# lars-frogner/Impact

Measured on AMD Instinct MI355X. Metric: voxels stepped/sec + remesh tris/sec, 512^3 grid, 1/2/4/8 MI355X, higher is better.
Workload: dtype i8 voxels, f32 SDF/mesh arithmetic, f64 moments; 1 GPU; config-2 SDF asteroid x2.05 -> 502^3 grid = 512^3 stored voxels (32768 chunks); parallelism=single GPU, voxels_per_gpu=134217728, regions=1, triangles=1813104

## Files before the change

impact_amd/csrc/sn_roles.hpp:

```cpp
#pragma once
#include "ivx_internal.hpp"

namespace ivx_roles {
namespace sn {


constexpr int G = 18, NROWS = 324, NCROWS = 289, NCUBES = 4913;
constexpr int RS = 24, TILE_BYTES = NROWS * RS;
constexpr uint32_t VPC = 864;
__device__ __forceinline__ int tix(int a, int b, int c) { return (a * G + b) * RS + 3 + c; }

__device__ __forceinline__ uint32_t opaque(uint32_t x) {
    asm volatile("" : "+v"(x));
    return x;
}
struct V3 {
    float x, y, z;
};
__device__ __forceinline__ V3 mk(float x, float y, float z) { return V3{x, y, z}; }
__device__ __forceinline__ V3 add(V3 a, V3 b) { return {a.x + b.x, a.y + b.y, a.z + b.z}; }
__device__ __forceinline__ V3 sub(V3 a, V3 b) { return {a.x - b.x, a.y - b.y, a.z - b.z}; }
__device__ __forceinline__ V3 mul(V3 a, V3 b) { return {a.x * b.x, a.y * b.y, a.z * b.z}; }
__device__ __forceinline__ V3 scale(V3 a, float s) { return {a.x * s, a.y * s, a.z * s}; }
__device__ __forceinline__ float len3(V3 a) { return sqrtf((a.x * a.x + a.y * a.y) + a.z * a.z); }
__device__ __forceinline__ bool sneg(float f) { return (__float_as_uint(f) >> 31) != 0; }
__device__ __forceinline__ float decode(int8_t e) { return (float)e * 0.02f; }

struct SnParams {
    GridView g;
    float extent;
    uint32_t x_off;
};

struct RowLoads {
    uint32_t c0, c1, c2;
    uint4 s4, t4;
    uint32_t b0s, b0t, b2s, b2t;
};
__device__ __forceinline__ uint32_t row_mode(const GridView& g, int gi, int gj) {
    if (gj < 0 || gj >= (int)g.cy * 16) return 0u;
    if (gi < 0 || gi >= (int)g.cx * 16) return 2u;
    return 1u;
}
__device__ __forceinline__ void row_issue(const GridView& g, int gi, int gj, int ck, RowLoads& L) {
    if (row_mode(g, gi, gj) != 1u) return;
    const size_t cidx = (size_t)(((gi >> 4) * g.cy + (gj >> 4)) * g.cz) + (size_t)ck;
    const uint32_t rix = (uint32_t)(((gi & 15) << 4) | (gj & 15));
    const size_t o = (cidx << 12) + ((size_t)rix << 4);
    const bool has_lo = ck > 0, has_hi = ck + 1 < (int)g.cz;
    const uint32_t* ip = reinterpret_cast<const uint32_t*>(g.info + cidx);
    const uint8_t* kf = g.kface + cidx * 1024 + rix;
    const uint32_t* ip0 = has_lo ? ip - 2 : ip;
    const uint32_t* ip2 = has_hi ? ip + 2 : ip;
    const uint8_t* kf0 = has_lo ? kf - 1024 : kf;
// ... 837 lines not shown
        if ((any & bit) == 0u) continue;
        const bool crossed = (cm & bit) != 0u;
        const float q = div_ranged(d[c1], d[c1] - d[c2]);
        const float t = crossed ? q : 0.0f;
        const float s = crossed ? ((1.0f - q) + q) : 0.0f;
        sum.x += axis == 4 ? t : ((c1 & 4) ? s : 0.0f);
        sum.y += axis == 2 ? t : ((c1 & 2) ? s : 0.0f);
        sum.z += axis == 1 ? t : ((c1 & 1) ? s : 0.0f);
    }
}

struct RowData {
    uint4 s4, t4;
    uint32_t b0s, b0t, b2s, b2t;
};
struct TileLoads {
    RowData L[2];
    uint32_t rec;
};
__device__ __forceinline__ void rim_row(int h, int& a, int& b) {
    a = h < 18 ? 0 : (h < 36 ? G - 1 : 1 + ((h - 36) >> 1));
    b = h < 18 ? h : (h < 36 ? h - 18 : ((h & 1) ? G - 1 : 0));
}
__device__ __forceinline__ void tile_issue(const GridView& g, uint32_t chunk, TileLoads& T, uint32_t tid) {
    tid = opaque(tid);
    const int ck = chunk % g.cz, cj = (chunk / g.cz) % g.cy, ci = chunk / (g.cz * g.cy);
    T.rec = 0u;
    if (tid < 27u) {
        const int di = (int)(tid / 9u) - 1, dj = (int)((tid / 3u) % 3u) - 1, dk = (int)(tid % 3u) - 1;
        const int ni = ci + di, nj = cj + dj, nk = ck + dk;
        if (nj >= 0 && nj < (int)g.cy && nk >= 0 && nk < (int)g.cz) {
            const ivx_chunk_info* rp = nullptr;
            if (ni >= 0 && ni < (int)g.cx) rp = g.info + (size_t)((ni * (int)g.cy + nj) * (int)g.cz + nk);
            else if (g.ghost_info[ni < 0 ? 0 : 1]) rp = g.ghost_info[ni < 0 ? 0 : 1] + (nj * (int)g.cz + nk);
            if (rp) T.rec = *reinterpret_cast<const uint32_t*>(rp);
        }
    }
    {
        RowData& L = T.L[0];
        const size_t o = ((size_t)chunk << 12) + ((size_t)tid << 4);
        const uint32_t* kf = reinterpret_cast<const uint32_t*>(g.kface + (size_t)chunk * 1024) + (tid >> 2);
        const uint32_t* kf0 = ck > 0 ? kf - 256 : kf;
        const uint32_t* kf2 = ck + 1 < (int)g.cz ? kf + 256 : kf;
        L.s4 = *reinterpret_cast<const uint4*>(g.sdf + o);
        L.t4 = *reinterpret_cast<const uint4*>(g.type + o);
        L.b0s = kf0[64];
        L.b0t = kf0[192];
        L.b2s = kf2[0];
        L.b2t = kf2[128];
    }
    {
        RowData& L = T.L[1];
        int a, b;
        rim_row((int)tid, a, b);
        int gi = ci * 16 + a - 1, gj = cj * 16 + b - 1;
        const bool real = tid < 68u && row_mode(g, gi, gj) == 1u;
        gi = real ? gi : ci * 16;
        gj = real ? gj : cj * 16;
        const size_t cidx = (size_t)(((gi >> 4) * g.cy + (gj >> 4)) * g.cz) + (size_t)ck;
        const uint32_t rix = (uint32_t)(((gi & 15) << 4) | (gj & 15));
        const size_t o = (cidx << 12) + ((size_t)rix << 4);
        const uint32_t* kf = reinterpret_cast<const uint32_t*>(g.kface + cidx * 1024) + (rix >> 2);
        const uint32_t* kf0 = ck > 0 ? kf - 256 : kf;
        const uint32_t* kf2 = ck + 1 < (int)g.cz ? kf + 256 : kf;
        L.s4 = *reinterpret_cast<const uint4*>(g.sdf + o);
        L.t4 = *reinterpret_cast<const uint4*>(g.type + o);
        L.b0s = kf0[64];
        L.b0t = kf0[192];
        L.b2s = kf2[0];
        L.b2t = kf2[128];
    }
}
__device__ __forceinline__ void tile_pin(TileLoads& T) {
#pragma unroll
    for (int r = 0; r < 2; ++r) {
        RowData& L = T.L[r];
        asm volatile("" : "+v"(L.s4.x), "+v"(L.s4.y), "+v"(L.s4.z), "+v"(L.s4.w), "+v"(L.t4.x), "+v"(L.t4.y), "+v"(L.t4.z), "+v"(L.t4.w));
        asm volatile("" : "+v"(L.b0s), "+v"(L.b0t), "+v"(L.b2s), "+v"(L.b2t));
    }
    asm volatile("" : "+v"(T.rec));
}
__device__ __forceinline__ void tile_records(TileLoads& T, uint32_t* s_rec, uint32_t tid) {
    if (tid < 27u) s_rec[tid] = T.rec;
}
__device__ __forceinline__ void tile_row_store(RowData& L, uint32_t rix, uint32_t w0, uint32_t w1, uint32_t w2, bool has_lo, bool has_hi, uint32_t sd[6],
                                               uint32_t ty[6]) {
    asm volatile("" : "+v"(L.s4.x), "+v"(L.s4.y), "+v"(L.s4.z), "+v"(L.s4.w), "+v"(L.t4.x), "+v"(L.t4.y), "+v"(L.t4.z), "+v"(L.t4.w));
    asm volatile("" : "+v"(L.b0s), "+v"(L.b0t), "+v"(L.b2s), "+v"(L.b2t));
    const ivx_chunk_info c0 = record_of(w0), c1 = record_of(w1), c2 = record_of(w2);
    const bool d1 = c1.kind == KIND_NONUNIFORM;
    const uint32_t us = ivx_uniform_sdf(c1.kind) * 0x01010101u, ut = ivx_uniform_type(c1) * 0x01010101u;
    sd[1] = d1 ? L.s4.x : us, sd[2] = d1 ? L.s4.y : us, sd[3] = d1 ? L.s4.z : us, sd[4] = d1 ? L.s4.w : us;
    ty[1] = d1 ? L.t4.x : ut, ty[2] = d1 ? L.t4.y : ut, ty[3] = d1 ? L.t4.z : ut, ty[4] = d1 ? L.t4.w : ut;
    const uint32_t sh = 8u * (rix & 3u);
    if (has_lo) {
        const bool dense = c0.kind == KIND_NONUNIFORM;
        sd[0] = dense ? ((L.b0s >> sh) & 0xFFu) : ivx_uniform_sdf(c0.kind);
        ty[0] = dense ? ((L.b0t >> sh) & 0xFFu) : ivx_uniform_type(c0);
    }
    if (has_hi) {
        const bool dense = c2.kind == KIND_NONUNIFORM;
        sd[5] = dense ? ((L.b2s >> sh) & 0xFFu) : ivx_uniform_sdf(c2.kind);
        ty[5] = dense ? ((L.b2t >> sh) & 0xFFu) : ivx_uniform_type(c2);
    }
}
__device__ __forceinline__ void tile_row_write(int r, const uint32_t sd[6], const uint32_t ty[6], uint8_t* s_sd, uint8_t* s_ty, uint32_t* s_neg) {
    s_neg[r] = ((sd[0] >> 7) & 1u) | (neg16(sd + 1) << 1) | (((sd[5] >> 7) & 1u) << 17);
    uint8_t* ds = s_sd + r * RS;
    uint8_t* dt = s_ty + r * RS;
    ds[3] = (uint8_t)sd[0];
    dt[3] = (uint8_t)ty[0];
#pragma unroll
    for (int q = 0; q < 4; ++q) {
        reinterpret_cast<uint32_t*>(ds + 4)[q] = sd[1 + q];
        reinterpret_cast<uint32_t*>(dt + 4)[q] = ty[1 + q];
    }
    ds[20] = (uint8_t)sd[5];
    dt[20] = (uint8_t)ty[5];
}
__device__ __forceinline__ void tile_finish(const GridView& g, uint32_t chunk, TileLoads& T, const uint32_t* s_rec, uint8_t* s_sd, uint8_t* s_ty, uint32_t* s_neg,
                                            uint32_t tid, int* upper) {
    tid = opaque(tid);
    const int ck = chunk % g.cz, cj = (chunk / g.cz) % g.cy, ci = chunk / (g.cz * g.cy);
    const bool has_lo = ck > 0, has_hi = ck + 1 < (int)g.cz;
    {
        uint32_t sd[6], ty[6];
        sd[0] = sd[5] = 0x7Fu;
        ty[0] = ty[5] = 0xFFu;
        tile_row_store(T.L[0], tid, s_rec[12], s_rec[13], s_rec[14], has_lo, has_hi, sd, ty);
        tile_row_write((int)(((tid >> 4) + 1u) * G + (tid & 15u) + 1u), sd, ty, s_sd, s_ty, s_neg);
    }
    if (tid < 68u) {
        int a, b;
        rim_row((int)tid, a, b);
        const int gi = ci * 16 + a - 1, gj = cj * 16 + b - 1;
        uint32_t sd[6], ty[6];
        sd[0] = sd[5] = 0x7Fu;
        ty[0] = ty[5] = 0xFFu;
        sd[1] = sd[2] = sd[3] = sd[4] = 0x7F7F7F7Fu;
        ty[1] = ty[2] = ty[3] = ty[4] = 0xFFFFFFFFu;
        const uint32_t mode = row_mode(g, gi, gj);
        if (mode == 2u) {
            fetch_row_serial(g, gi, gj, ck, sd, ty);
        } else if (mode == 1u) {
            const int col = (((gi >> 4) - ci + 1) * 3 + ((gj >> 4) - cj + 1)) * 3;
            tile_row_store(T.L[1], (uint32_t)(((gi & 15) << 4) | (gj & 15)), s_rec[col], s_rec[col + 1], s_rec[col + 2], has_lo, has_hi, sd, ty);
        }
        tile_row_write(a * G + b, sd, ty, s_sd, s_ty, s_neg);
    }
    upper[0] = upper[1] = upper[2] = G - 1;
    if ((s_rec[22] & 0xFFu) == KIND_NONUNIFORM) upper[0] -= 1;
    if ((s_rec[16] & 0xFFu) == KIND_NONUNIFORM) upper[1] -= 1;
    if ((s_rec[14] & 0xFFu) == KIND_NONUNIFORM) upper[2] -= 1;
}

static inline uint32_t ivx_emit_grid(const ivx_grid* g, uint32_t n_entries) {
    const uint32_t resident = (uint32_t)g->ctx->n_cu * 4u;
    return n_entries < resident ? (n_entries ? n_entries : 1u) : resident;
}
static inline uint32_t ivx_emit_general_grid(const ivx_grid* g, uint32_t n_entries) {
    const uint32_t cap = (uint32_t)g->ctx->n_cu * 2u;
    return n_entries < cap ? (n_entries ? n_entries : 1u) : cap;
}

#define IVX_MESH_ST(p, v) __builtin_nontemporal_store((v), (p))
template <bool SLOTS>
__device__ __forceinline__ void role_sn_emit(uint32_t bid, uint32_t nb, SnParams p, float* __restrict__ positions, float* __restrict__ normals,
                                                 uint32_t* __restrict__ indices, unsigned long long* __restrict__ imats, ivx_submesh* __restrict__ submeshes,
                                                 const uint32_t* __restrict__ emit_count, const uint4* __restrict__ emit_items, uint32_t vcap, uint32_t icap,
                                                 uint32_t scap, const uint32_t* __restrict__ slots, uint32_t* __restrict__ hard_count,
                                                 uint32_t* __restrict__ hard_list, uint32_t* __restrict__ cursor, SnWalk walk = SnWalk{nullptr, nullptr, nullptr, 0u},
                                                 uint32_t walk_len = 0u) {
    __shared__ uint16_t s_quad[3 * VPC];
    __shared__ __attribute__((aligned(16))) uint8_t s_sd[TILE_BYTES];
    __shared__ __attribute__((aligned(16))) uint8_t s_ty[TILE_BYTES];
    __shared__ uint32_t s_neg2[2][NROWS];
    __shared__ uint32_t s_vrow[NCROWS];
    __shared__ uint16_t s_qrow[NCROWS];
    __shared__ uint2 s_qbits[NCROWS];
    __shared__ uint32_t s_nq;
    __shared__ uint16_t s_surf[VPC];
    __shared__ float s_vpos[3][VPC];
    __shared__ uint8_t s_vsm[VPC];
    __shared__ uint32_t s_wsum[4];
    __shared__ uint32_t s_hard;
    __shared__ uint32_t s_rec[27];
    __shared__ uint32_t s_ticket[5];
    __shared__ float s_rcount[13];
    const GridView& g = p.g;
    const uint32_t tid = threadIdx.x;
    if (tid >= 1u && tid < 13u) s_rcount[tid] = 1.0f / (float)tid;
    const uint32_t n_emit = emit_count[0];
    constexpr uint32_t NONE = 0xFFFFFFFFu;
    const uint32_t walk_front = walk.items ? walk.count[0] : 0u;
    uint32_t li = NONE, li_next = bid, li_prev = NONE;
    if (li_next >= n_emit) return;
    uint4 item = make_uint4(0u, 0u, 0u, 0u), item_next;
    if (walk.items) {
        const uint32_t w = bid < walk_front ? bid : walk_len - 1u - (bid - walk_front);
        item_next = walk.items[w];
        li_next = walk.li[w];
    } else {
        item_next = emit_items[li_next];
    }
    int upper[3] = {G - 1, G - 1, G - 1};
    uint32_t info_w = 0u;
// ... 17 lines not shown
        sm.chunk_indices[0] = (uint32_t)ci + p.x_off;
        sm.chunk_indices[1] = (uint32_t)cj;
        sm.chunk_indices[2] = (uint32_t)ck;
        sm.index_offset = ioff;
        sm.index_count = icount;
        for (int a = 0; a < 2; ++a)
            for (int b = 0; b < 2; ++b)
                for (int c = 0; c < 2; ++c)
                    sm.is_obscured_from_direction[a][b][c] =
                        (((cflags >> (3 * a)) & 1u) && ((cflags >> (3 * b + 1)) & 1u) && ((cflags >> (3 * c + 2)) & 1u)) ? 1u : 0u;
        sm.vertex_offset = voff;
        sm.vertex_count = item.w & 0xFFFFu;
        sm.reserved = 0;
        submeshes[slot] = sm;
    }
    __syncthreads();
    if (have) IVX_T(g, li, 1);
    if (from_ticket) {
        li_next = (uint32_t)__builtin_amdgcn_readfirstlane((int)s_ticket[0]);
        item_next = make_uint4((uint32_t)__builtin_amdgcn_readfirstlane((int)s_ticket[1]), (uint32_t)__builtin_amdgcn_readfirstlane((int)s_ticket[2]),
                               (uint32_t)__builtin_amdgcn_readfirstlane((int)s_ticket[3]), (uint32_t)__builtin_amdgcn_readfirstlane((int)s_ticket[4]));
    }
    const bool have_next = li_next < n_emit;
    if (tid == 0) {
        if (li_prev != NONE && s_hard) hard_list[atomicAdd(hard_count, 1u)] = li_prev;
        s_hard = large ? 1u : 0u;
    }

    uint32_t ticket = 0u;
    if (tid == TK && have_next) ticket = nb + 8u * atomicAdd(cursor + 32u * (bid & 7u), 1u) + (bid & 7u);
    TileLoads T;
    if (have_next) tile_issue(g, item_next.x, T, tid);
    uint4 drawn = make_uint4(0u, 0u, 0u, 0u);
    uint32_t drawn_li = 0u;
    {
        uint32_t vb[2] = {0, 0}, nq[2] = {0, 0};
        const int r0 = 2 * (int)opaque(tid);
        for (int q = 0; q < 2; ++q) {
            const int cr = r0 + q;
            if (cr < NCROWS) {
                uint32_t qx, qy, qz;
                cube_row_bits(s_neg, cr / 17, cr % 17, upper, vb[q], qx, qy, qz);
                nq[q] = __popc(qx) + __popc(qy) + __popc(qz);
                s_qbits[cr] = make_uint2(qx | (qy << 17), (qy >> 15) | (qz << 2));
            }
        }
        uint32_t total;
        const uint32_t pre = block_prefix<false>((__popc(vb[0]) + __popc(vb[1])) | ((nq[0] + nq[1]) << 16), s_wsum, tid, total);
        uint32_t base = pre & 0xFFFFu, qb = pre >> 16;
        if (tid == 0) s_nq = total >> 16;
        for (int q = 0; q < 2; ++q) {
            const int cr = r0 + q;
            if (cr < NCROWS) {
                s_vrow[cr] = (base << 17) | vb[q];
                s_qrow[cr] = (uint16_t)qb;
                qb += nq[q];
                uint32_t m = vb[q];
                while (m) {
                    const int k = __ffs(m) - 1;
                    m &= m - 1;
                    if (base < VPC) s_surf[base] = (uint16_t)(cr * 17 + k);
                    base += 1;
                }
            }
        }
    }
    if (have_next) tile_pin(T);
    if (have) IVX_T(g, li, 6);
    __syncthreads();
    if (have) IVX_T(g, li, 2);
    if ((tid >> 6) == (TK >> 6)) {
        const uint32_t tk = (uint32_t)__builtin_amdgcn_readfirstlane((int)ticket);
        if (have_next && tk < n_emit) {
            if (walk.items) {
                const uint32_t w = tk < walk_front ? tk : walk_len - 1u - (tk - walk_front);
                drawn = walk.items[w];
                drawn_li = walk.li[w];
            } else {
                drawn = emit_items[tk];
                drawn_li = tk;
            }
            asm volatile("" : "+v"(drawn.x), "+v"(drawn.y), "+v"(drawn.z), "+v"(drawn.w), "+v"(drawn_li));
        } else {
            drawn_li = tk;
        }
    }

    const float chunk_extent = p.extent * 16.0f;
    const V3 pos_offset = mk((float)(ci + (int)p.x_off) * chunk_extent - 0.5f * p.extent, (float)cj * chunk_extent - 0.5f * p.extent,
                             (float)ck * chunk_extent - 0.5f * p.extent);

    for (uint32_t v0 = (uint32_t)__builtin_amdgcn_readfirstlane((int)(tid & ~63u)); v0 < vcount; v0 += 256) {
        const uint32_t v_raw = v0 + (opaque(tid) & 63u);
        const bool v_live = v_raw < vcount;
        const uint32_t v = v_live ? v_raw : vcount - 1u;
        const int cid = s_surf[v];
        const int cr = cid / 17, k = cid - cr * 17, i = cr / 17, j = cr - i * 17;
        const int t0 = tix(i, j, k);
        const int co[8] = {0, 1, RS, RS + 1, G * RS, G * RS + 1, G * RS + RS, G * RS + RS + 1};
        float d[8];
        uint32_t neg = 0u;
        uint8_t mats[8];
#pragma unroll
        for (int c = 0; c < 8; ++c) {
            const int8_t e = (int8_t)s_sd[t0 + co[c]];
            d[c] = decode(e);
            neg |= (e < 0 ? 1u : 0u) << c;
            mats[c] = s_ty[t0 + co[c]];
        }
        int count;
        V3 sum;
        edge_centroid(d, neg, sum, count);
        const float rc = s_rcount[count];
        const V3 centroid = scale(sum, rc);
        const V3 d00 = sub(mk(d[4], d[2], d[1]), mk(d[0], d[0], d[0]));
        const V3 d01 = sub(mk(d[5], d[6], d[3]), mk(d[1], d[4], d[2]));
        const V3 d10 = sub(mk(d[6], d[3], d[5]), mk(d[2], d[1], d[4]));
        const V3 d11 = sub(mk(d[7], d[7], d[7]), mk(d[3], d[5], d[6]));
        const V3 o = centroid;
        const V3 r = sub(mk(1.0f, 1.0f, 1.0f), o);
        const V3 r_yzx = mk(r.y, r.z, r.x), r_zxy = mk(r.z, r.x, r.y), o_yzx = mk(o.y, o.z, o.x), o_zxy = mk(o.z, o.x, o.y);
        const V3 grad = add(add(add(mul(mul(r_yzx, r_zxy), d00), mul(mul(r_yzx, o_zxy), d01)), mul(mul(o_yzx, r_zxy), d10)),
                            mul(mul(o_yzx, o_zxy), d11));
        const float gl2 = (grad.x * grad.x + grad.y * grad.y) + grad.z * grad.z;
        V3 normal;
        if (__builtin_amdgcn_ballot_w64(!(gl2 >= 0x1p-100f)) == 0ull) {
            normalize_ranged(grad.x, grad.y, grad.z, gl2, normal.x, normal.y, normal.z);
        } else {
            const float gl = sqrtf(gl2);
            normal = mk(grad.x / gl, grad.y / gl, grad.z / gl);
        }
        const V3 position = add(scale(add(centroid, mk((float)i, (float)j, (float)k)), p.extent), pos_offset);
        uint32_t m0 = 0xFFFFFFFFu;
        bool single = true;
#pragma unroll
        for (int c = 0; c < 8; ++c)
            if ((neg >> c) & 1u) {
                if (m0 == 0xFFFFFFFFu) m0 = mats[c];
                single = single && mats[c] == m0;
            }
        const uint2 qb = s_qbits[cr];
        const uint32_t below = (1u << k) - 1u;
        const uint32_t qslot0 = (uint32_t)s_qrow[cr] + __popc(qb.x & (below | (below << 17))) + __popc(qb.y & ((below >> 15) | (below << 2)));
        if (v_live) {
            const size_t gv = (size_t)voff + v;
            IVX_MESH_ST(positions + 3 * gv + 0, position.x);
            IVX_MESH_ST(positions + 3 * gv + 1, position.y);
            IVX_MESH_ST(positions + 3 * gv + 2, position.z);
            IVX_MESH_ST(normals + 3 * gv + 0, normal.x);
            IVX_MESH_ST(normals + 3 * gv + 1, normal.y);
            IVX_MESH_ST(normals + 3 * gv + 2, normal.z);
            s_vpos[0][v] = position.x;
            s_vpos[1][v] = position.y;
            s_vpos[2][v] = position.z;
            s_vsm[v] = (uint8_t)m0;
            if (!single) s_hard = 1u;
            uint32_t qslot = qslot0;
            if ((qb.x >> k) & 1u) s_quad[qslot++] = (uint16_t)cid;
            if (k < 15 ? ((qb.x >> (17 + k)) & 1u) : ((qb.y >> (k - 15)) & 1u)) s_quad[qslot++] = (uint16_t)(cid | (1 << 13));
            if ((qb.y >> (2 + k)) & 1u) s_quad[qslot] = (uint16_t)(cid | (2 << 13));
        }
    }
    if (have) IVX_T(g, li, 7);
    if (have_next) tile_records(T, s_rec, tid);
    __syncthreads();
    if (have) IVX_T(g, li, 3);


    if (vcount && !s_hard) {
        const uint32_t n_quads = s_nq;
        for (uint32_t q0 = (uint32_t)__builtin_amdgcn_readfirstlane((int)(tid & ~63u)); q0 < n_quads; q0 += 256) {
            const uint32_t lane = opaque(tid) & 63u;
            const uint32_t q_raw = q0 + lane;
            const bool q_live = q_raw < n_quads;
            const uint32_t q = q_live ? q_raw : n_quads - 1u;
            const uint32_t qd = s_quad[q];
            const int axis = (int)(qd >> 13);
            const int qcid = (int)(qd & 0x1FFFu);
            const int cr = qcid / 17;
            const int k = qcid - cr * 17, i = cr / 17, j = cr - i * 17;
            const int ab = axis == 0 ? 17 : (axis == 1 ? 1 : 289);
            const int ac = axis == 0 ? 1 : (axis == 1 ? 289 : 17);
            const bool n1 = ((s_neg[i * G + j] >> k) & 1u) != 0u;
            const bool negative_face = !n1;
            const int rb = ab == 1 ? 0 : (ab == 17 ? 1 : 17), rc = ac == 1 ? 0 : (ac == 17 ? 1 : 17);
            const int kb = ab == 1 ? 1 : 0, kc = ac == 1 ? 1 : 0;
            const uint32_t v1 = vertex_of(s_vrow[cr], k), v2 = vertex_of(s_vrow[cr - rb], k - kb), v3 = vertex_of(s_vrow[cr - rc], k - kc),
                           v4 = vertex_of(s_vrow[cr - rb - rc], k - kb - kc);
            const V3 q1 = mk(s_vpos[0][v1], s_vpos[1][v1], s_vpos[2][v1]), q2 = mk(s_vpos[0][v2], s_vpos[1][v2], s_vpos[2][v2]);
            const V3 q3 = mk(s_vpos[0][v3], s_vpos[1][v3], s_vpos[2][v3]), q4 = mk(s_vpos[0][v4], s_vpos[1][v4], s_vpos[2][v4]);
            const uint32_t b1 = s_vsm[v1], b2 = s_vsm[v2], b3 = s_vsm[v3], b4 = s_vsm[v4];
            uint32_t quad[6];
            const V3 e14 = sub(q1, q4), e23 = sub(q2, q3);
            const float sq14 = (e14.x * e14.x + e14.y * e14.y) + e14.z * e14.z, sq23 = (e23.x * e23.x + e23.y * e23.y) + e23.z * e23.z;
            bool first = sq14 < sq23;
            if (__builtin_amdgcn_ballot_w64(first) != 0ull) first = sqrtf(sq14) < sqrtf(sq23);
            if (first) {
                if (negative_face) { quad[0] = v1; quad[1] = v4; quad[2] = v2; quad[3] = v1; quad[4] = v3; quad[5] = v4; }
                else { quad[0] = v1; quad[1] = v2; quad[2] = v4; quad[3] = v1; quad[4] = v4; quad[5] = v3; }
            } else if (negative_face) { quad[0] = v2; quad[1] = v3; quad[2] = v4; quad[3] = v2; quad[4] = v1; quad[5] = v3; }
            else { quad[0] = v2; quad[1] = v4; quad[2] = v3; quad[3] = v2; quad[4] = v3; quad[5] = v1; }
            if (q_live) {
                const size_t io = (size_t)ioff + (size_t)q * 6;
#pragma unroll
                for (int t = 0; t < 6; ++t) IVX_MESH_ST(indices + io + t, voff + quad[t]);
                if (!(b1 == b2 && b1 == b3 && b1 == b4)) s_hard = 1u;
            }
            const uint32_t rem3 = 3u * min(n_quads - q0, 64u);
            uint4* imw = reinterpret_cast<uint4*>(imats + (size_t)ioff + (size_t)q0 * 6);
#pragma unroll
            for (int jx = 0; jx < 3; ++jx) {
                const uint32_t x = lane + 64u * (uint32_t)jx;
                const uint32_t src = (x * 171u) >> 9;
                const uint32_t bm = (uint32_t)__builtin_amdgcn_ds_bpermute((int)(src << 2), (int)b1);
                if (x < rem3) {
                    uint32_t* w_ = reinterpret_cast<uint32_t*>(imw + x);
                    IVX_MESH_ST(w_, bm), IVX_MESH_ST(w_ + 1, 1u), IVX_MESH_ST(w_ + 2, bm), IVX_MESH_ST(w_ + 3, 1u);
                }
            }
        }
    }
    if (tid == TK && have_next) {
        s_ticket[0] = ticket < n_emit ? drawn_li : NONE;
        s_ticket[1] = drawn.x, s_ticket[2] = drawn.y, s_ticket[3] = drawn.z, s_ticket[4] = drawn.w;
    }
    if (have) IVX_T(g, li, 4);

    if (have_next) {
        tile_finish(g, item_next.x, T, s_rec, s_sd, s_ty, s_neg2[buf ^ 1u], tid, upper);
        info_w = s_rec[13];
    }
    if (have) IVX_T(g, li, 5);
    if (!have_next) break;
    li_prev = li;
    li = li_next;
    item = item_next;
    from_ticket = true;
    buf ^= 1u;
    }
    __syncthreads();
    if (tid == 0 && li != NONE && s_hard) hard_list[atomicAdd(hard_count, 1u)] = li;
}

template <bool SLOTS>
__device__ __forceinline__ void role_sn_emit_general(uint32_t bid, uint32_t nb, SnParams p, float* __restrict__ positions, float* __restrict__ normals,
                                                 uint32_t* __restrict__ indices, unsigned long long* __restrict__ imats,
                                                 uint4* __restrict__ vmats, ivx_submesh* __restrict__ submeshes, const uint32_t* __restrict__ emit_count,
                                                 const uint4* __restrict__ emit_items, uint32_t vcap, uint32_t icap, uint32_t scap,
                                                 const uint32_t* __restrict__ slots, const uint32_t* __restrict__ hard_count,
                                                 const uint32_t* __restrict__ hard_list) {
    __shared__ uint16_t s_quad[768];
    __shared__ __attribute__((aligned(16))) uint8_t s_sd[TILE_BYTES];
// ... 256 lines not shown
```

impact_amd/csrc/step_fused.hip:

```cpp
#include "ccl_roles.hpp"
#include "sn_roles.hpp"
#include "table_roles.hpp"
#include "many.hpp"

namespace {
using namespace ivx_roles;

struct StepArgs {
    GridView g;
    float extent;
    uint32_t x_off;
    uint32_t n_chunks;
    uint32_t nb[6];
    const uint8_t* flags;
    uint8_t* labels;
    ivx_chunk_info* info;
    uint32_t* rparent;
    uint32_t* rcompid;
    uint32_t* rscalar;
    uint32_t* multi_list;
    uint32_t* ccl_group_sums;
    const uint8_t* touch;
    uint32_t* counts;
    uint32_t* sn_group_sums;
// ... 20 lines not shown
    double* partials;
    uint32_t n_partials;
    double* moments_out;
    uint32_t* host_block;
    const uint32_t* eval_count;
    uint32_t count_run;
    uint32_t x_part;
    uint32_t seq;
    uint32_t fp_side, fp_cap;
    const uint16_t* fp_nbr;
    uint32_t* fp_count;
    uint2* fp_pairs;
    uint32_t* fp_seen;
    unsigned long long* record;
    uint32_t record_max_pairs;
    unsigned long long* record_head;
    uint32_t record_head_words;
    sn::BoxNeeds needs_box;
    const uint32_t* needs_touched;
    uint32_t* needs_out;
    uint32_t* needs_early;
    uint32_t* needs_counter;
    uint32_t* needs_bell;
    uint32_t needs_seq, pad_needs_;
    const uint32_t* copy_src;
    uint32_t* copy_dst;
    uint32_t copy_words;
};

__device__ __forceinline__ sn::SnParams sn_params(const StepArgs& a) {
    sn::SnParams p;
    p.g = a.g;
    p.extent = a.extent;
    p.x_off = a.x_off;
    return p;
}

__device__ __forceinline__ void step_post1_body(const StepArgs& a, uint32_t b, uint32_t) {
    __shared__ uint32_t sh_words[4 * sn::NROWS + 16];
    struct { uint32_t* par; } sh{sh_words};
    if (b < a.nb[1]) {
        role_ccl_merge_columns(b, a.nb[1], a.g, a.touch, a.rparent);
        return;
    }
    b -= a.nb[1];
    if (b < a.nb[0]) {
        if (b == 0u && threadIdx.x < 2u && a.walk.items) a.walk.count[threadIdx.x] = 0u;
        sn::role_sn_count_waves(b, a.nb[0], sn_params(a), a.counts, a.sn_group_sums, a.work_count, a.active_list, sh.par, a.count_run, a.x_part);
        return;
    }
    b -= a.nb[0];
    if (b < a.nb[3]) {
        role_occupied_partial(b, a.g.cx, a.g.cy, a.g.cz, a.bbox, a.occ_part);
        return;
    }
    b -= a.nb[3];
    if (b < a.nb[4]) {
// ... 53 lines not shown
    if (b < a.nb[1]) {
        sn::role_sn_scan(b, a.nb[1], a.n_chunks, a.counts, a.sn_group_sums, a.offsets, a.ranks, a.emit_items, a.walk);
        return;
    }
    b -= a.nb[1];
    if (b < a.nb[2]) {
        role_inertia_final(a.n_partials, a.extent, a.partials, a.moments_out);
        return;
    }
    b -= a.nb[2];
    if (b < a.nb[3]) {
        role_occupied_final(a.n_occ_slots, a.occ_part, a.rscalar + 16);
        return;
    }
    b -= a.nb[3];
    if (b < a.nb[4]) {
        __shared__ uint32_t s_seen[128];
        role_face_pairs(b, a.g, a.fp_side, a.labels, a.rcompid, a.fp_nbr, a.fp_count, a.fp_pairs, a.fp_cap, a.fp_seen, s_seen);
    }
}
__global__ __launch_bounds__(256) void k_step_post2(StepArgs a) { step_post2_body(a, blockIdx.x, gridDim.x); }
IVX_MANY_TWIN(k_step_post2_many, StepArgs, step_post2_body, __launch_bounds__(256))

__device__ __forceinline__ void step_emit_body(const StepArgs& a, uint32_t b, uint32_t) {
    if (b < a.nb[0]) {
        role_ccl_flatten(b, a.nb[0], a.g, a.rparent, a.multi_list , a.ccl_group_sums);
        return;
    }
    b -= a.nb[0];
    if (b < a.nb[1]) {
        sn::role_sn_emit<false>(b, a.nb[1], sn_params(a), a.positions, a.normals, a.indices, a.imats, a.submeshes, a.offsets + 2 * (size_t)a.n_chunks + 2,
                                a.emit_items, a.vcap, a.icap, a.scap, nullptr, a.hard_count, a.hard_list, a.hard_count + 32, a.walk, a.n_chunks);
        return;
    }
    b -= a.nb[1];
    if (b < a.nb[2]) {
        role_step_record(a.rscalar, a.fp_count, a.fp_pairs, a.offsets + 2 * (size_t)a.n_chunks, a.moments_out, a.x_off, a.record_max_pairs, a.record);
        if (a.record_head) {
            __syncthreads();
            for (uint32_t i = threadIdx.x; i < a.record_head_words; i += 256u) a.record_head[i] = a.record[i];
        }
        if (threadIdx.x < 64u) role_result_gather(a.rscalar, a.offsets + 2 * (size_t)a.n_chunks, a.moments_out, a.work_count, a.eval_count, a.host_block, false, 0u);
    }
}
__global__ __launch_bounds__(256) __attribute__((amdgpu_waves_per_eu(4, 4))) void k_step_emit(StepArgs a) { step_emit_body(a, blockIdx.x, gridDim.x); }
IVX_MANY_TWIN(k_step_emit_many, StepArgs, step_emit_body, __launch_bounds__(256) __attribute__((amdgpu_waves_per_eu(4, 4))))

__device__ __forceinline__ void step_assign_body(const StepArgs& a, uint32_t b, uint32_t) {
    if (b < a.nb[0]) {
        role_ccl_assign<true>(b, a.nb[0], a.g, a.rparent, a.multi_list , a.ccl_group_sums, a.nb[0], a.rcompid, a.rscalar);
        return;
    }
    sn::role_sn_emit_general<false>(b - a.nb[0], a.nb[1], sn_params(a), a.positions, a.normals, a.indices, a.imats, a.vmats, a.submeshes,
                                    a.offsets + 2 * (size_t)a.n_chunks + 2, a.emit_items, a.vcap, a.icap, a.scap, nullptr, a.hard_count, a.hard_list);
}
__global__ __launch_bounds__(256) __attribute__((amdgpu_waves_per_eu(4, 4))) void k_step_assign(StepArgs a) { step_assign_body(a, blockIdx.x, gridDim.x); }
IVX_MANY_TWIN(k_step_assign_many, StepArgs, step_assign_body, __launch_bounds__(256) __attribute__((amdgpu_waves_per_eu(4, 4))))

__device__ __forceinline__ void step_gather_body(const StepArgs& a, uint32_t, uint32_t) {
    role_result_gather(a.rscalar, a.offsets + 2 * (size_t)a.n_chunks, a.moments_out, a.work_count, a.eval_count, a.host_block, false, 0u);
    for (uint32_t i0 = threadIdx.x; i0 < a.copy_words; i0 += 512u) {
        uint32_t v[8];
#pragma unroll
        for (uint32_t q = 0; q < 8u; ++q) v[q] = i0 + 64u * q < a.copy_words ? a.copy_src[i0 + 64u * q] : 0u;
#pragma unroll
        for (uint32_t q = 0; q < 8u; ++q)
            if (i0 + 64u * q < a.copy_words) a.copy_dst[i0 + 64u * q] = v[q];
    }
    __threadfence_system();
// ... 140 lines not shown
        a.nb[4] = (g->cc[1] * g->cc[2] + FACE_COLS - 1u) / FACE_COLS;
    }
    const uint32_t groups = (g->n_chunks + 255u) / 256u;
    if (stages & IVX_STAGE_REGIONS) {
        a.nb[0] = g->n_chunks < 64u ? g->n_chunks : 64u;
        const uint32_t want = g->n_chunks / 16u;
        a.nb[5] = want < 8u ? (g->n_chunks < 8u ? g->n_chunks : 8u) : (want > 128u ? 128u : want);
    }
    if (stages & IVX_STAGE_REMESH) a.nb[1] = groups;
    if (stages & IVX_STAGE_INERTIA) {
        a.nb[2] = 1;
        a.n_partials = groups < (uint32_t)g->partial_blocks ? groups : (uint32_t)g->partial_blocks;
    }
    if (stages & IVX_STAGE_OCCUPIED) a.nb[3] = 1;
    const uint32_t total = a.nb[0] + a.nb[1] + a.nb[2] + a.nb[3] + a.nb[4] + a.nb[5];
    if (total == 0) return IVX_OK;
    if (!ivx_many_try(g->ctx, g, IVX_MK_POST2, total, a)) IVX_KLAUNCH(k_step_post2, dim3(total), dim3(256), 0, g->ctx->stream, a);
    IVX_HIP_CHECK(hipGetLastError());
    return IVX_OK;
}

int ivx_launch_step_emit(ivx_grid* g, uint32_t stages, bool general_in_assign, void* slab_record, bool record_has_pairs) {
    StepArgs a = make_args(g);
    if (stages & IVX_STAGE_REGIONS) a.nb[0] = (g->n_chunks + 255u) / 256u;
    if (stages & IVX_STAGE_REMESH) {
        a.nb[1] = sn::ivx_emit_grid(g, g->n_chunks);
        g->sn_tail_zero = 0;
    }
    if (slab_record) {
        face_pair_args(a, g, record_has_pairs ? reinterpret_cast<const uint16_t*>(g->pairs_dev)  : nullptr);
        a.record = static_cast<unsigned long long*>(slab_record);
        a.record_max_pairs = IVX_MAX_FACE_PAIRS;
        a.record_head = g->record_head_copy;
        a.record_head_words = g->record_head_words;
        a.nb[2] = 1;
    }
    const uint32_t total = a.nb[0] + a.nb[1] + a.nb[2];
    if (total == 0) return IVX_OK;
    if (!ivx_many_try(g->ctx, g, IVX_MK_EMIT, total, a)) IVX_KLAUNCH(k_step_emit, dim3(total), dim3(256), 0, g->ctx->stream, a);
    IVX_HIP_CHECK(hipGetLastError());
    if ((stages & IVX_STAGE_REMESH) && !general_in_assign) return ivx_launch_sn_emit_general(g);
    return IVX_OK;
}

bool ivx_step_assign_fits(const ivx_grid* g) { return (g->n_chunks + 255u) / 256u <= ASSIGN_MAX_GROUPS; }

int ivx_launch_step_assign(ivx_grid* g, bool with_mesher_general, bool with_ccl) {
    StepArgs a = make_args(g);
    a.nb[0] = with_ccl ? (g->n_chunks + 255u) / 256u : 0u;
    a.nb[1] = with_mesher_general ? sn::ivx_emit_general_grid(g, g->n_chunks) : 0u;
    if (a.nb[0] + a.nb[1] == 0u) return IVX_OK;
    if (!ivx_many_try(g->ctx, g, IVX_MK_ASSIGN, a.nb[0] + a.nb[1], a)) IVX_KLAUNCH(k_step_assign, dim3(a.nb[0] + a.nb[1]), dim3(256), 0, g->ctx->stream, a);
    IVX_HIP_CHECK(hipGetLastError());
    return IVX_OK;
}

int ivx_launch_step_gather(ivx_grid* g) {
    StepArgs a = make_args(g);
    a.seq = ++g->result_seq;
    a.copy_src = g->gather_copy_src, a.copy_dst = g->gather_copy_dst, a.copy_words = g->gather_copy_words;
    g->gather_copy_words = 0;
    if (!ivx_many_try(g->ctx, g, IVX_MK_GATHER, 1u, a)) IVX_KLAUNCH(k_step_gather, dim3(1), dim3(64), 0, g->ctx->stream, a);
// ... 10 lines not shown
```

impact_amd/csrc/surface_nets.hip:

```cpp
#include "sn_roles.hpp"
#include "many.hpp"

namespace {
using namespace ivx_roles::sn;

__global__ __launch_bounds__(256) void k_sn_count(SnParams p, uint32_t* __restrict__ counts, uint32_t* __restrict__ group_sums,
                                                  const uint32_t* __restrict__ work_counts, const uint32_t* __restrict__ active_list, uint32_t run) {
    __shared__ uint32_t s_rows[4 * NROWS];
    role_sn_count_waves(blockIdx.x, gridDim.x, p, counts, group_sums, work_counts, active_list, s_rows, run);
}
__global__ __launch_bounds__(256) void k_sn_scan(uint32_t n_chunks, const uint32_t* __restrict__ counts, const uint32_t* __restrict__ group_sums,
                                                 uint32_t* __restrict__ offsets, uint32_t* __restrict__ ranks, uint4* __restrict__ emit_items) {
    role_sn_scan(blockIdx.x, gridDim.x, n_chunks, counts, group_sums, offsets, ranks, emit_items);
}
template <bool SLOTS>
__global__ __launch_bounds__(256) __attribute__((amdgpu_waves_per_eu(4, 4))) void k_sn_emit(SnParams p, float* __restrict__ positions, float* __restrict__ normals,
                                                 uint32_t* __restrict__ indices, unsigned long long* __restrict__ imats, ivx_submesh* __restrict__ submeshes,
                                                 const uint32_t* __restrict__ emit_count, const uint4* __restrict__ emit_items, uint32_t vcap, uint32_t icap,
                                                 uint32_t scap, const uint32_t* __restrict__ slots, uint32_t* __restrict__ hard_count,
                                                 uint32_t* __restrict__ hard_list, uint32_t* __restrict__ cursor) {
    role_sn_emit<SLOTS>(blockIdx.x, gridDim.x, p, positions, normals, indices, imats, submeshes, emit_count, emit_items, vcap, icap, scap, slots, hard_count, hard_list,
                        cursor);
}
template <bool SLOTS>
// ... 114 lines not shown

}

int ivx_selftest_mesher_division(ivx_ctx* ctx, uint32_t* mismatches) {
    IVX_REQUIRE(ctx && mismatches, IVX_ERR_INVALID, "ivx_selftest_mesher_division: null argument");
    uint32_t* d = nullptr;
    IVX_HIP_CHECK(hipMalloc(&d, sizeof(uint32_t)));
    IVX_HIP_CHECK(ivx_memset_async(d, 0, sizeof(uint32_t), ctx->stream));
    IVX_KLAUNCH(k_selftest_division, dim3(257), dim3(256), 0, ctx->stream, d);
    IVX_HIP_CHECK(hipGetLastError());
    IVX_KLAUNCH(k_selftest_normalize, dim3(65536), dim3(256), 0, ctx->stream, d);
    IVX_HIP_CHECK(hipGetLastError());
    IVX_HIP_CHECK(ivx_memcpy_async(mismatches, d, sizeof(uint32_t), hipMemcpyDeviceToHost, ctx->stream));
    IVX_HIP_CHECK(ivx_stream_sync(ctx->stream));
    IVX_HIP_CHECK(hipFree(d));
    return IVX_OK;
}

static SnParams make_params(ivx_grid* g) {
    SnParams p;
    p.g = ivx_view(g);
    p.extent = g->extent;
    p.x_off = g->x_off;
    return p;
}

int ivx_launch_sn_count(ivx_grid* g) {
    if (int rc_l = ivx_ensure_active_list(g)) return rc_l;
    const uint32_t groups = (g->n_chunks + 255u) / 256u;
    uint32_t* gs = g->group_sums + groups;
    IVX_HIP_CHECK(ivx_memset_async(gs, 0, sizeof(uint32_t) * (IVX_SN_GROUP_WORDS * groups + IVX_SN_TAIL_WORDS), g->ctx->stream));
    g->scratch_dirty |= IVX_SCRATCH_SN;
    g->preset_fresh &= ~IVX_SCRATCH_SN;
    const uint32_t run = ivx_count_run(g);
    IVX_KLAUNCH(k_sn_count, dim3((ivx_list_grid(g) + 4u * run - 1u) / (4u * run)), dim3(256), 0, g->ctx->stream, make_params(g), g->chunk_counts, gs, ivx_wc(g),
                       g->active_list, run);
    IVX_HIP_CHECK(hipGetLastError());
    return IVX_OK;
}

int ivx_launch_box_mesh_needs(ivx_grid* g, const uint32_t t_lo[3], const uint32_t t_cc[3], const uint32_t b_lo[3], const uint32_t b_cc[3], const uint32_t* d_touched,
                              uint32_t* d_out) {
    BoxNeeds bx;
    for (int d = 0; d < 3; ++d) bx.t_lo[d] = t_lo[d], bx.t_cc[d] = t_cc[d], bx.b_lo[d] = b_lo[d], bx.b_cc[d] = b_cc[d];
    const uint32_t n = b_cc[0] * b_cc[1] * b_cc[2];
    if (n == 0) return IVX_OK;
// ... 68 lines not shown
```

Measured before the change: 741.7 billion voxels/s.

## Add single-type specialization of surface-nets emit skipping type loads and LDS

Adds a template specialization of the surface-nets emit path for grids known to hold a single voxel type. It drops the per-voxel type loads, type LDS tile, per-vertex material tracking and mixed-material checks, and uses a ballot over neighbour records to send any chunk with a different uniform type to the hard list. With the LDS and VGPR footprint smaller, the specialized kernel targets more waves per EU and launches a larger emit grid, and rim-row loads are now skipped for waves past the first two. Correctness depends on the signs_type/signs_current host flags staying accurate.

```diff
diff --git a/impact_amd/csrc/sn_roles.hpp b/impact_amd/csrc/sn_roles.hpp
--- a/impact_amd/csrc/sn_roles.hpp
+++ b/impact_amd/csrc/sn_roles.hpp
@@ -30,6 +30,7 @@
     GridView g;
     float extent;
     uint32_t x_off;
+    uint32_t single_type;
 };
 
 struct RowLoads {
@@ -913,6 +914,7 @@
     a = h < 18 ? 0 : (h < 36 ? G - 1 : 1 + ((h - 36) >> 1));
     b = h < 18 ? h : (h < 36 ? h - 18 : ((h & 1) ? G - 1 : 0));
 }
+template <bool ST>
 __device__ __forceinline__ void tile_issue(const GridView& g, uint32_t chunk, TileLoads& T, uint32_t tid) {
     tid = opaque(tid);
     const int ck = chunk % g.cz, cj = (chunk / g.cz) % g.cy, ci = chunk / (g.cz * g.cy);
@@ -934,13 +936,15 @@
         const uint32_t* kf0 = ck > 0 ? kf - 256 : kf;
         const uint32_t* kf2 = ck + 1 < (int)g.cz ? kf + 256 : kf;
         L.s4 = *reinterpret_cast<const uint4*>(g.sdf + o);
-        L.t4 = *reinterpret_cast<const uint4*>(g.type + o);
         L.b0s = kf0[64];
-        L.b0t = kf0[192];
         L.b2s = kf2[0];
-        L.b2t = kf2[128];
-    }
-    {
+        if constexpr (!ST) {
+            L.t4 = *reinterpret_cast<const uint4*>(g.type + o);
+            L.b0t = kf0[192];
+            L.b2t = kf2[128];
+        }
+    }
+    if ((uint32_t)__builtin_amdgcn_readfirstlane((int)tid) < 128u) {
         RowData& L = T.L[1];
         int a, b;
         rim_row((int)tid, a, b);
@@ -955,60 +959,70 @@
         const uint32_t* kf0 = ck > 0 ? kf - 256 : kf;
         const uint32_t* kf2 = ck + 1 < (int)g.cz ? kf + 256 : kf;
         L.s4 = *reinterpret_cast<const uint4*>(g.sdf + o);
-        L.t4 = *reinterpret_cast<const uint4*>(g.type + o);
         L.b0s = kf0[64];
-        L.b0t = kf0[192];
         L.b2s = kf2[0];
-        L.b2t = kf2[128];
-    }
-}
+        if constexpr (!ST) {
+            L.t4 = *reinterpret_cast<const uint4*>(g.type + o);
+            L.b0t = kf0[192];
+            L.b2t = kf2[128];
+        }
+    }
+}
+template <bool ST>
 __device__ __forceinline__ void tile_pin(TileLoads& T) {
 #pragma unroll
     for (int r = 0; r < 2; ++r) {
         RowData& L = T.L[r];
-        asm volatile("" : "+v"(L.s4.x), "+v"(L.s4.y), "+v"(L.s4.z), "+v"(L.s4.w), "+v"(L.t4.x), "+v"(L.t4.y), "+v"(L.t4.z), "+v"(L.t4.w));
-        asm volatile("" : "+v"(L.b0s), "+v"(L.b0t), "+v"(L.b2s), "+v"(L.b2t));
+        asm volatile("" : "+v"(L.s4.x), "+v"(L.s4.y), "+v"(L.s4.z), "+v"(L.s4.w), "+v"(L.b0s), "+v"(L.b2s));
+        if constexpr (!ST) asm volatile("" : "+v"(L.t4.x), "+v"(L.t4.y), "+v"(L.t4.z), "+v"(L.t4.w), "+v"(L.b0t), "+v"(L.b2t));
     }
     asm volatile("" : "+v"(T.rec));
 }
 __device__ __forceinline__ void tile_records(TileLoads& T, uint32_t* s_rec, uint32_t tid) {
     if (tid < 27u) s_rec[tid] = T.rec;
 }
+template <bool ST>
 __device__ __forceinline__ void tile_row_store(RowData& L, uint32_t rix, uint32_t w0, uint32_t w1, uint32_t w2, bool has_lo, bool has_hi, uint32_t sd[6],
                                                uint32_t ty[6]) {
-    asm volatile("" : "+v"(L.s4.x), "+v"(L.s4.y), "+v"(L.s4.z), "+v"(L.s4.w), "+v"(L.t4.x), "+v"(L.t4.y), "+v"(L.t4.z), "+v"(L.t4.w));
-    asm volatile("" : "+v"(L.b0s), "+v"(L.b0t), "+v"(L.b2s), "+v"(L.b2t));
+    asm volatile("" : "+v"(L.s4.x), "+v"(L.s4.y), "+v"(L.s4.z), "+v"(L.s4.w), "+v"(L.b0s), "+v"(L.b2s));
+    if constexpr (!ST) asm volatile("" : "+v"(L.t4.x), "+v"(L.t4.y), "+v"(L.t4.z), "+v"(L.t4.w), "+v"(L.b0t), "+v"(L.b2t));
     const ivx_chunk_info c0 = record_of(w0), c1 = record_of(w1), c2 = record_of(w2);
     const bool d1 = c1.kind == KIND_NONUNIFORM;
-    const uint32_t us = ivx_uniform_sdf(c1.kind) * 0x01010101u, ut = ivx_uniform_type(c1) * 0x01010101u;
+    const uint32_t us = ivx_uniform_sdf(c1.kind) * 0x01010101u;
     sd[1] = d1 ? L.s4.x : us, sd[2] = d1 ? L.s4.y : us, sd[3] = d1 ? L.s4.z : us, sd[4] = d1 ? L.s4.w : us;
-    ty[1] = d1 ? L.t4.x : ut, ty[2] = d1 ? L.t4.y : ut, ty[3] = d1 ? L.t4.z : ut, ty[4] = d1 ? L.t4.w : ut;
+    if constexpr (!ST) {
+        const uint32_t ut = ivx_uniform_type(c1) * 0x01010101u;
+        ty[1] = d1 ? L.t4.x : ut, ty[2] = d1 ? L.t4.y : ut, ty[3] = d1 ? L.t4.z : ut, ty[4] = d1 ? L.t4.w : ut;
+    }
     const uint32_t sh = 8u * (rix & 3u);
     if (has_lo) {
         const bool dense = c0.kind == KIND_NONUNIFORM;
         sd[0] = dense ? ((L.b0s >> sh) & 0xFFu) : ivx_uniform_sdf(c0.kind);
-        ty[0] = dense ? ((L.b0t >> sh) & 0xFFu) : ivx_uniform_type(c0);
+        if constexpr (!ST) ty[0] = dense ? ((L.b0t >> sh) & 0xFFu) : ivx_uniform_type(c0);
     }
     if (has_hi) {
         const bool dense = c2.kind == KIND_NONUNIFORM;
         sd[5] = dense ? ((L.b2s >> sh) & 0xFFu) : ivx_uniform_sdf(c2.kind);
-        ty[5] = dense ? ((L.b2t >> sh) & 0xFFu) : ivx_uniform_type(c2);
-    }
-}
+        if constexpr (!ST) ty[5] = dense ? ((L.b2t >> sh) & 0xFFu) : ivx_uniform_type(c2);
+    }
+}
+template <bool ST>
 __device__ __forceinline__ void tile_row_write(int r, const uint32_t sd[6], const uint32_t ty[6], uint8_t* s_sd, uint8_t* s_ty, uint32_t* s_neg) {
     s_neg[r] = ((sd[0] >> 7) & 1u) | (neg16(sd + 1) << 1) | (((sd[5] >> 7) & 1u) << 17);
     uint8_t* ds = s_sd + r * RS;
-    uint8_t* dt = s_ty + r * RS;
     ds[3] = (uint8_t)sd[0];
-    dt[3] = (uint8_t)ty[0];
-#pragma unroll
-    for (int q = 0; q < 4; ++q) {
-        reinterpret_cast<uint32_t*>(ds + 4)[q] = sd[1 + q];
-        reinterpret_cast<uint32_t*>(dt + 4)[q] = ty[1 + q];
-    }
+#pragma unroll
+    for (int q = 0; q < 4; ++q) reinterpret_cast<uint32_t*>(ds + 4)[q] = sd[1 + q];
     ds[20] = (uint8_t)sd[5];
-    dt[20] = (uint8_t)ty[5];
-}
+    if constexpr (!ST) {
+        uint8_t* dt = s_ty + r * RS;
+        dt[3] = (uint8_t)ty[0];
+#pragma unroll
+        for (int q = 0; q < 4; ++q) reinterpret_cast<uint32_t*>(dt + 4)[q] = ty[1 + q];
+        dt[20] = (uint8_t)ty[5];
+    }
+}
+template <bool ST>
 __device__ __forceinline__ void tile_finish(const GridView& g, uint32_t chunk, TileLoads& T, const uint32_t* s_rec, uint8_t* s_sd, uint8_t* s_ty, uint32_t* s_neg,
                                             uint32_t tid, int* upper) {
     tid = opaque(tid);
@@ -1018,8 +1032,8 @@
         uint32_t sd[6], ty[6];
         sd[0] = sd[5] = 0x7Fu;
         ty[0] = ty[5] = 0xFFu;
-        tile_row_store(T.L[0], tid, s_rec[12], s_rec[13], s_rec[14], has_lo, has_hi, sd, ty);
-        tile_row_write((int)(((tid >> 4) + 1u) * G + (tid & 15u) + 1u), sd, ty, s_sd, s_ty, s_neg);
+        tile_row_store<ST>(T.L[0], tid, s_rec[12], s_rec[13], s_rec[14], has_lo, has_hi, sd, ty);
+        tile_row_write<ST>((int)(((tid >> 4) + 1u) * G + (tid & 15u) + 1u), sd, ty, s_sd, s_ty, s_neg);
     }
     if (tid < 68u) {
         int a, b;
@@ -1035,9 +1049,9 @@
             fetch_row_serial(g, gi, gj, ck, sd, ty);
         } else if (mode == 1u) {
             const int col = (((gi >> 4) - ci + 1) * 3 + ((gj >> 4) - cj + 1)) * 3;
-            tile_row_store(T.L[1], (uint32_t)(((gi & 15) << 4) | (gj & 15)), s_rec[col], s_rec[col + 1], s_rec[col + 2], has_lo, has_hi, sd, ty);
-        }
-        tile_row_write(a * G + b, sd, ty, s_sd, s_ty, s_neg);
+            tile_row_store<ST>(T.L[1], (uint32_t)(((gi & 15) << 4) | (gj & 15)), s_rec[col], s_rec[col + 1], s_rec[col + 2], has_lo, has_hi, sd, ty);
+        }
+        tile_row_write<ST>(a * G + b, sd, ty, s_sd, s_ty, s_neg);
     }
     upper[0] = upper[1] = upper[2] = G - 1;
     if ((s_rec[22] & 0xFFu) == KIND_NONUNIFORM) upper[0] -= 1;
@@ -1045,8 +1059,11 @@
     if ((s_rec[14] & 0xFFu) == KIND_NONUNIFORM) upper[2] -= 1;
 }
 
-static inline uint32_t ivx_emit_grid(const ivx_grid* g, uint32_t n_entries) {
-    const uint32_t resident = (uint32_t)g->ctx->n_cu * 4u;
+#ifndef IVX_EMIT_ST_PER_CU
+#define IVX_EMIT_ST_PER_CU 5
+#endif
+static inline uint32_t ivx_emit_grid(const ivx_grid* g, uint32_t n_entries, uint32_t per_cu = 4u) {
+    const uint32_t resident = (uint32_t)g->ctx->n_cu * per_cu;
     return n_entries < resident ? (n_entries ? n_entries : 1u) : resident;
 }
 static inline uint32_t ivx_emit_general_grid(const ivx_grid* g, uint32_t n_entries) {
@@ -1055,7 +1072,7 @@
 }
 
 #define IVX_MESH_ST(p, v) __builtin_nontemporal_store((v), (p))
-template <bool SLOTS>
+template <bool SLOTS, bool ST = false>
 __device__ __forceinline__ void role_sn_emit(uint32_t bid, uint32_t nb, SnParams p, float* __restrict__ positions, float* __restrict__ normals,
                                                  uint32_t* __restrict__ indices, unsigned long long* __restrict__ imats, ivx_submesh* __restrict__ submeshes,
                                                  const uint32_t* __restrict__ emit_count, const uint4* __restrict__ emit_items, uint32_t vcap, uint32_t icap,
@@ -1064,7 +1081,7 @@
                                                  uint32_t walk_len = 0u) {
     __shared__ uint16_t s_quad[3 * VPC];
     __shared__ __attribute__((aligned(16))) uint8_t s_sd[TILE_BYTES];
-    __shared__ __attribute__((aligned(16))) uint8_t s_ty[TILE_BYTES];
+    __shared__ __attribute__((aligned(16))) uint8_t s_ty[ST ? 16 : TILE_BYTES];
     __shared__ uint32_t s_neg2[2][NROWS];
     __shared__ uint32_t s_vrow[NCROWS];
     __shared__ uint16_t s_qrow[NCROWS];
@@ -1072,7 +1089,7 @@
     __shared__ uint32_t s_nq;
     __shared__ uint16_t s_surf[VPC];
     __shared__ float s_vpos[3][VPC];
-    __shared__ uint8_t s_vsm[VPC];
+    __shared__ uint8_t s_vsm[ST ? 4 : VPC];
     __shared__ uint32_t s_wsum[4];
     __shared__ uint32_t s_hard;
     __shared__ uint32_t s_rec[27];
@@ -1136,15 +1153,22 @@
                                (uint32_t)__builtin_amdgcn_readfirstlane((int)s_ticket[3]), (uint32_t)__builtin_amdgcn_readfirstlane((int)s_ticket[4]));
     }
     const bool have_next = li_next < n_emit;
+    bool other_type = false;
+    if constexpr (ST) {
+        if (tid < 64u) {
+            const uint32_t w = tid < 27u ? s_rec[tid] : 0u;
+            other_type = __builtin_amdgcn_ballot_w64((w & 0xFFu) == KIND_UNIFORM && (w >> 24) != p.single_type) != 0ull;
+        }
+    }
     if (tid == 0) {
         if (li_prev != NONE && s_hard) hard_list[atomicAdd(hard_count, 1u)] = li_prev;
-        s_hard = large ? 1u : 0u;
+        s_hard = (large || other_type) ? 1u : 0u;
     }
 
     uint32_t ticket = 0u;
     if (tid == TK && have_next) ticket = nb + 8u * atomicAdd(cursor + 32u * (bid & 7u), 1u) + (bid & 7u);
     TileLoads T;
-    if (have_next) tile_issue(g, item_next.x, T, tid);
+    if (have_next) tile_issue<ST>(g, item_next.x, T, tid);
     uint4 drawn = make_uint4(0u, 0u, 0u, 0u);
     uint32_t drawn_li = 0u;
     {
@@ -1179,7 +1203,7 @@
             }
         }
     }
-    if (have_next) tile_pin(T);
+    tile_pin<ST>(T);
     if (have) IVX_T(g, li, 6);
     __syncthreads();
     if (have) IVX_T(g, li, 2);
@@ -1214,13 +1238,13 @@
         const int co[8] = {0, 1, RS, RS + 1, G * RS, G * RS + 1, G * RS + RS, G * RS + RS + 1};
         float d[8];
         uint32_t neg = 0u;
-        uint8_t mats[8];
+        [[maybe_unused]] uint8_t mats[8];
 #pragma unroll
         for (int c = 0; c < 8; ++c) {
             const int8_t e = (int8_t)s_sd[t0 + co[c]];
             d[c] = decode(e);
             neg |= (e < 0 ? 1u : 0u) << c;
-            mats[c] = s_ty[t0 + co[c]];
+            if constexpr (!ST) mats[c] = s_ty[t0 + co[c]];
         }
         int count;
         V3 sum;
@@ -1245,14 +1269,16 @@
             normal = mk(grad.x / gl, grad.y / gl, grad.z / gl);
         }
         const V3 position = add(scale(add(centroid, mk((float)i, (float)j, (float)k)), p.extent), pos_offset);
-        uint32_t m0 = 0xFFFFFFFFu;
+        uint32_t m0 = ST ? p.single_type : 0xFFFFFFFFu;
         bool single = true;
-#pragma unroll
-        for (int c = 0; c < 8; ++c)
-            if ((neg >> c) & 1u) {
-                if (m0 == 0xFFFFFFFFu) m0 = mats[c];
-                single = single && mats[c] == m0;
-            }
+        if constexpr (!ST) {
+#pragma unroll
+            for (int c = 0; c < 8; ++c)
+                if ((neg >> c) & 1u) {
+                    if (m0 == 0xFFFFFFFFu) m0 = mats[c];
+                    single = single && mats[c] == m0;
+                }
+        }
         const uint2 qb = s_qbits[cr];
         const uint32_t below = (1u << k) - 1u;
         const uint32_t qslot0 = (uint32_t)s_qrow[cr] + __popc(qb.x & (below | (below << 17))) + __popc(qb.y & ((below >> 15) | (below << 2)));
@@ -1267,8 +1293,10 @@
             s_vpos[0][v] = position.x;
             s_vpos[1][v] = position.y;
             s_vpos[2][v] = position.z;
-            s_vsm[v] = (uint8_t)m0;
-            if (!single) s_hard = 1u;
+            if constexpr (!ST) {
+                s_vsm[v] = (uint8_t)m0;
+                if (!single) s_hard = 1u;
+            }
             uint32_t qslot = qslot0;
             if ((qb.x >> k) & 1u) s_quad[qslot++] = (uint16_t)cid;
             if (k < 15 ? ((qb.x >> (17 + k)) & 1u) : ((qb.y >> (k - 15)) & 1u)) s_quad[qslot++] = (uint16_t)(cid | (1 << 13));
@@ -1303,7 +1331,7 @@
                            v4 = vertex_of(s_vrow[cr - rb - rc], k - kb - kc);
             const V3 q1 = mk(s_vpos[0][v1], s_vpos[1][v1], s_vpos[2][v1]), q2 = mk(s_vpos[0][v2], s_vpos[1][v2], s_vpos[2][v2]);
             const V3 q3 = mk(s_vpos[0][v3], s_vpos[1][v3], s_vpos[2][v3]), q4 = mk(s_vpos[0][v4], s_vpos[1][v4], s_vpos[2][v4]);
-            const uint32_t b1 = s_vsm[v1], b2 = s_vsm[v2], b3 = s_vsm[v3], b4 = s_vsm[v4];
+            const uint32_t b1 = ST ? p.single_type : s_vsm[v1], b2 = ST ? b1 : s_vsm[v2], b3 = ST ? b1 : s_vsm[v3], b4 = ST ? b1 : s_vsm[v4];
             uint32_t quad[6];
             const V3 e14 = sub(q1, q4), e23 = sub(q2, q3);
             const float sq14 = (e14.x * e14.x + e14.y * e14.y) + e14.z * e14.z, sq23 = (e23.x * e23.x + e23.y * e23.y) + e23.z * e23.z;
@@ -1341,7 +1369,7 @@
     if (have) IVX_T(g, li, 4);
 
     if (have_next) {
-        tile_finish(g, item_next.x, T, s_rec, s_sd, s_ty, s_neg2[buf ^ 1u], tid, upper);
+        tile_finish<ST>(g, item_next.x, T, s_rec, s_sd, s_ty, s_neg2[buf ^ 1u], tid, upper);
         info_w = s_rec[13];
     }
     if (have) IVX_T(g, li, 5);
diff --git a/impact_amd/csrc/step_fused.hip b/impact_amd/csrc/step_fused.hip
--- a/impact_amd/csrc/step_fused.hip
+++ b/impact_amd/csrc/step_fused.hip
@@ -66,7 +66,8 @@
     uint32_t* needs_early;
     uint32_t* needs_counter;
     uint32_t* needs_bell;
-    uint32_t needs_seq, pad_needs_;
+    uint32_t needs_seq;
+    uint32_t single_type;
     const uint32_t* copy_src;
     uint32_t* copy_dst;
     uint32_t copy_words;
@@ -77,6 +78,7 @@
     p.g = a.g;
     p.extent = a.extent;
     p.x_off = a.x_off;
+    p.single_type = a.single_type;
     return p;
 }
 
@@ -176,6 +178,7 @@
 __global__ __launch_bounds__(256) void k_step_post2(StepArgs a) { step_post2_body(a, blockIdx.x, gridDim.x); }
 IVX_MANY_TWIN(k_step_post2_many, StepArgs, step_post2_body, __launch_bounds__(256))
 
+template <bool ST>
 __device__ __forceinline__ void step_emit_body(const StepArgs& a, uint32_t b, uint32_t) {
     if (b < a.nb[0]) {
         role_ccl_flatten(b, a.nb[0], a.g, a.rparent, a.multi_list , a.ccl_group_sums);
@@ -183,7 +186,7 @@
     }
     b -= a.nb[0];
     if (b < a.nb[1]) {
-        sn::role_sn_emit<false>(b, a.nb[1], sn_params(a), a.positions, a.normals, a.indices, a.imats, a.submeshes, a.offsets + 2 * (size_t)a.n_chunks + 2,
+        sn::role_sn_emit<false, ST>(b, a.nb[1], sn_params(a), a.positions, a.normals, a.indices, a.imats, a.submeshes, a.offsets + 2 * (size_t)a.n_chunks + 2,
                                 a.emit_items, a.vcap, a.icap, a.scap, nullptr, a.hard_count, a.hard_list, a.hard_count + 32, a.walk, a.n_chunks);
         return;
     }
@@ -197,8 +200,9 @@
         if (threadIdx.x < 64u) role_result_gather(a.rscalar, a.offsets + 2 * (size_t)a.n_chunks, a.moments_out, a.work_count, a.eval_count, a.host_block, false, 0u);
     }
 }
-__global__ __launch_bounds__(256) __attribute__((amdgpu_waves_per_eu(4, 4))) void k_step_emit(StepArgs a) { step_emit_body(a, blockIdx.x, gridDim.x); }
-IVX_MANY_TWIN(k_step_emit_many, StepArgs, step_emit_body, __launch_bounds__(256) __attribute__((amdgpu_waves_per_eu(4, 4))))
+template <bool ST>
+__global__ __launch_bounds__(256) __attribute__((amdgpu_waves_per_eu(ST ? IVX_EMIT_ST_PER_CU : 4, ST ? IVX_EMIT_ST_PER_CU : 4))) void k_step_emit(StepArgs a) { step_emit_body<ST>(a, blockIdx.x, gridDim.x); }
+IVX_MANY_TWIN(k_step_emit_many, StepArgs, step_emit_body<false>, __launch_bounds__(256) __attribute__((amdgpu_waves_per_eu(4, 4))))
 
 __device__ __forceinline__ void step_assign_body(const StepArgs& a, uint32_t b, uint32_t) {
     if (b < a.nb[0]) {
@@ -385,9 +389,11 @@
 
 int ivx_launch_step_emit(ivx_grid* g, uint32_t stages, bool general_in_assign, void* slab_record, bool record_has_pairs) {
     StepArgs a = make_args(g);
+    const bool single_type = g->signs_current && !g->has_ghost[0] && !g->has_ghost[1] && !ivx_many_recording();
+    a.single_type = g->signs_type;
     if (stages & IVX_STAGE_REGIONS) a.nb[0] = (g->n_chunks + 255u) / 256u;
     if (stages & IVX_STAGE_REMESH) {
-        a.nb[1] = sn::ivx_emit_grid(g, g->n_chunks);
+        a.nb[1] = sn::ivx_emit_grid(g, g->n_chunks, single_type ? IVX_EMIT_ST_PER_CU : 4u);
         g->sn_tail_zero = 0;
     }
     if (slab_record) {
@@ -400,7 +406,8 @@
     }
     const uint32_t total = a.nb[0] + a.nb[1] + a.nb[2];
     if (total == 0) return IVX_OK;
-    if (!ivx_many_try(g->ctx, g, IVX_MK_EMIT, total, a)) IVX_KLAUNCH(k_step_emit, dim3(total), dim3(256), 0, g->ctx->stream, a);
+    if (single_type) IVX_KLAUNCH(k_step_emit<true>, dim3(total), dim3(256), 0, g->ctx->stream, a);
+    else if (!ivx_many_try(g->ctx, g, IVX_MK_EMIT, total, a)) IVX_KLAUNCH(k_step_emit<false>, dim3(total), dim3(256), 0, g->ctx->stream, a);
     IVX_HIP_CHECK(hipGetLastError());
     if ((stages & IVX_STAGE_REMESH) && !general_in_assign) return ivx_launch_sn_emit_general(g);
     return IVX_OK;
diff --git a/impact_amd/csrc/surface_nets.hip b/impact_amd/csrc/surface_nets.hip
--- a/impact_amd/csrc/surface_nets.hip
+++ b/impact_amd/csrc/surface_nets.hip
@@ -160,6 +160,7 @@
     p.g = ivx_view(g);
     p.extent = g->extent;
     p.x_off = g->x_off;
+    p.single_type = 0xFFu;
     return p;
 }
 
```

Result: faster. 780.3 billion voxels/s, median of 6 (+5.2%).
